# slimgroup/SetIntersectionProjection.jl

Measured on AMD Instinct MI355X. Metric: PARSDMM iterations/sec, higher is better.
Workload: dtype f32

## Files before the change

### setintersectionprojection.jl_amd/csrc/kernels_proj.hip

```cpp
#include <cstdlib>
#include <cstring>
#include <stdexcept>
#include <string>
#include <type_traits>

#include "sipx_device.h"

namespace sipx {

#if defined(__HIP_DEVICE_COMPILE__) && !defined(__gfx950__)
#error "kernels_proj.hip: the relaxed-atomics hand-offs assume gfx950 (see the comment above); port them to release/acquire first"
#endif

constexpr double L1_CAP = 131072.0;
constexpr int L1_REFINES = 1;
constexpr int L1_REFINES_SLAB = 6;
#ifndef SIPX_SPEC_CAP
#define SIPX_SPEC_CAP 1024
#endif
constexpr int SPEC_CAP = SIPX_SPEC_CAP;
constexpr double L1_HW_MAX = 1e-2;
constexpr double L1_CAPDIV = 64.0;
constexpr int L1_WIN_LO = 3, L1_WIN_HI = 4;
__device__ __forceinline__ double l1_probe_mult(int k) {
  const double m[L1_K] = {-64.0, -16.0, -4.0, -1.0, 1.0, 4.0, 16.0, 64.0};
  return m[k];
}
#define SIPX_PASS_GRID launch_blocks(5)
constexpr int SL_ABOVE_S = PREP_SLOTS, SL_ABOVE_C = PREP_SLOTS + 1;
enum { M_FIRST = 0, M_PROBE = 1, M_COMPACT = 2, M_DIST = 3, M_STORE = 4 ,
       M_LEAN = 5  };

template <typename T, int V, int MODE, int SRC>
__global__ __launch_bounds__(BLOCK) void k_pass(Grid G, SetArgs<T> a, int v_is_s, const T* __restrict__ varr,
                                                long long len, ProjScalars<T>* ps, T* __restrict__ compact,
                                                double* __restrict__ partials, T* __restrict__ maxpart) {
  if (MODE == M_PROBE && !(ps->need && !ps->spec_ok && ps->refine)) return;
  long long* cidx = nullptr;
  if (MODE == M_COMPACT && a.prox == PX_CARD) cidx = ps->cidx;
  if (MODE == M_COMPACT && !(ps->need && !ps->spec_ok)) return;
  constexpr bool GATHERS = MODE == M_FIRST || MODE == M_COMPACT || MODE == M_LEAN;
  __shared__ T sbuf[GATHERS ? SPEC_CAP : 1];
  __shared__ unsigned int scnt, sused;
  __shared__ int sovf;
  __shared__ unsigned long long sbase;
  double acc[PREP_SLOTS];
#pragma unroll
  for (int k = 0; k < PREP_SLOTS; ++k) acc[k] = 0;
  ProbeAcc<T> pa;
  if ((a.prox == PX_L1 || a.prox == PX_CARD) && (MODE <= M_PROBE || MODE == M_LEAN)) {
#pragma unroll
    for (int k = 0; k < L1_K; ++k) pa.t[k] = (T)ps->t[k];
  }
  double r_lo = 0, r_hi = -1;
  if ((MODE == M_FIRST || MODE == M_LEAN) && a.prox == PX_L1 && !(a.flags & F_NOSPEC)) { r_lo = ps->spec_lo; r_hi = ps->spec_hi; }
  if (MODE == M_COMPACT) { r_lo = ps->lo; r_hi = ps->hi; }
  const bool gather = r_hi > r_lo;
  const bool lean = (MODE == M_FIRST || MODE == M_LEAN) && a.prox == PX_L1 && gather && ps->lean != 0;
  if (MODE == M_FIRST && lean) return;
  if (MODE == M_LEAN && !lean) return;
  T vmax = T(0), vminp = (T)INFINITY;
  if (GATHERS) {
    if (threadIdx.x == 0) { scnt = 0; sused = 0; sovf = 0; }
    __syncthreads();
  }
  ProxCtx<T> pc;
  if (MODE == M_DIST) pc = make_prox<T>(a.prox, a.plo, a.phi, T(0), ps);
  const int lane = threadIdx.x & 63;

  auto body = [&](T x, long long e, bool live) {
    const T av = fabs(x);
    const double ad = (double)av;
    if (MODE == M_LEAN) {
      pa.add_lean(av, L1_WIN_LO, L1_WIN_HI);
      vminp = (av > T(0) && av < vminp) ? av : vminp;
    } else if (MODE == M_FIRST || MODE == M_PROBE) {
      pa.add(av, x);
      vmax = av > vmax ? av : vmax;
      if (MODE == M_FIRST) vminp = (av > T(0) && av < vminp) ? av : vminp;
    }
    if (MODE == M_COMPACT && ad > r_hi) {
      acc[0] += ad;
      acc[1] += 1.0;
    }
    if (MODE == M_STORE && live) compact[e] = x;
    if (MODE == M_DIST && live) {
      const T pv = prox_apply<T>(pc, x, T(0), T(0), T(0), e);
      const T dlt = pv - x;
      acc[0] += (double)dlt * (double)dlt;
      acc[1] += (double)x * (double)x;
    }
    if (GATHERS && gather) {
      const bool in = ad > r_lo && ad <= r_hi;
      const unsigned long long mask = __ballot(in);
      if (mask) {
        const int leader = __ffsll((long long)mask) - 1;
        const int cnt = __popcll(mask);
        const int my = __popcll(mask & ((1ull << lane) - 1ull));
        unsigned int base = SPEC_CAP;
        if (!cidx) {
          if (lane == leader) base = atomicAdd(&scnt, (unsigned int)cnt);
          base = __shfl(base, leader, 64);
        }
        if (cidx) {
          unsigned long long gb = 0;
          if (lane == leader) gb = atomicAdd(&ps->n_compact, (unsigned long long)cnt);
          gb = __shfl(gb, leader, 64);
          if (in) { compact[gb + my] = av; cidx[gb + my] = e; }
        } else if (base + cnt <= SPEC_CAP) {
          if (in) sbuf[base + my] = av;
          if (lane == leader) atomicMax(&sused, base + (unsigned int)cnt);
        } else if (MODE == M_FIRST || MODE == M_LEAN) {
          sovf = 1;
        } else {
          unsigned long long gb = 0;
          if (lane == leader) gb = atomicAdd(&ps->n_compact, (unsigned long long)cnt);
          gb = __shfl(gb, leader, 64);
          if (in) compact[gb + my] = av;
        }
      }
    }
  };

  auto drain = [&]() {
    if (MODE != M_COMPACT || !gather || cidx) return;
    __syncthreads();
    if (scnt <= SPEC_CAP / 2) return;
    const unsigned int cnt = sused;
    if (threadIdx.x == 0) sbase = cnt ? atomicAdd(&ps->n_compact, (unsigned long long)cnt) : 0ull;
    __syncthreads();
    for (unsigned int i = threadIdx.x; i < cnt; i += BLOCK) compact[sbase + i] = sbuf[i];
    __syncthreads();
    if (threadIdx.x == 0) { scnt = 0; sused = 0; }
    __syncthreads();
  };
  if (SRC == 0) {
    int round = 0;
    for (long long e0 = (long long)blockIdx.x * BLOCK; e0 < len; e0 += (long long)gridDim.x * BLOCK) {
      const long long e = e0 + threadIdx.x;
      body(e < len ? varr[e] : T(0), e, e < len);
      if ((++round & 3) == 0) drain();
    }
  } else {
    const bool ident = a.nblk == 0;
    const int nb = ident ? 1 : a.nblk;
    const bool relax = !(a.gamma == T(1));
    const T gam = a.gamma, omg = T(1) - a.gamma;
    long long v0, nvec;
    vec_range<V>(G, v0, nvec);
    const long long nit = (nvec - v0 + (long long)gridDim.x * BLOCK - 1) / ((long long)gridDim.x * BLOCK);
    for (long long it = 0; it < nit; ++it) {
      const long long vi = v0 + it * (long long)gridDim.x * BLOCK + (long long)blockIdx.x * BLOCK + threadIdx.x;
      const bool live = vi < nvec;
      const long long g = live ? vi * V : v0 * V;
      const Coord c = coords(G, g);
      const Vec<T, V> xc = ldv<T, V>(a.x + g);
      for (int q = 0; q < nb; ++q) {
        const long long e = (long long)q * G.N + g;
        T s[V];
        bool valid[V];
        if (ident) {
#pragma unroll
          for (int k = 0; k < V; ++k) { s[k] = xc.v[k]; valid[k] = true; }
        } else {
          fwd_dir<T, V>(G, a.x, xc, g, c, a.dir[q], a.ih[q], s, valid);
        }
        T out[V];
        if (v_is_s) {
#pragma unroll
          for (int k = 0; k < V; ++k) out[k] = s[k];
        } else {
          const Vec<T, V> yv = ldv<T, V>(a.y + e), lv = ldv<T, V>(a.l + e);
#pragma unroll
          for (int k = 0; k < V; ++k) {
            const T xh = relax ? (gam * s[k] + omg * yv.v[k]) : s[k];
            out[k] = valid[k] ? (xh - lv.v[k] * a.rho1) : T(0);
          }
        }
#pragma unroll
        for (int k = 0; k < V; ++k) body(live ? out[k] : T(0), e + k, live);
      }
      drain();
    }
  }

  if (MODE == M_FIRST || MODE == M_PROBE) {
    pa.to_slots(acc);
    block_reduce_store<PREP_SLOTS>(acc, partials, 0);
    if (MODE == M_FIRST) {
      block_max_store<T>(vmax, maxpart);
      block_min_store<T>(vminp, maxpart + NB);
    }
  } else if (MODE == M_LEAN) {
    double a5[5] = {pa.asum, pa.S[L1_WIN_LO], pa.S[L1_WIN_HI], (double)pa.C[L1_WIN_LO], (double)pa.C[L1_WIN_HI]};
    const int slots[5] = {0, 3 + L1_WIN_LO, 3 + L1_WIN_HI, 3 + L1_K + L1_WIN_LO, 3 + L1_K + L1_WIN_HI};
    block_reduce_store_at<5>(a5, partials, slots);
    block_min_store<T>(vminp, maxpart + NB);
  } else if (MODE == M_COMPACT) {
    double a2[2] = {acc[0], acc[1]};
    block_reduce_store<2>(a2, partials, SL_ABOVE_S);
  } else if (MODE == M_STORE) {
  } else {
    double a2[2] = {acc[0], acc[1]};
    block_reduce_store<2>(a2, partials, 0);
  }
  if (GATHERS && gather) {
    __syncthreads();
    const unsigned int cnt = sused;
    if (threadIdx.x == 0) {
      sbase = cnt ? atomicAdd(&ps->n_compact, (unsigned long long)cnt) : 0ull;
      if ((MODE == M_FIRST || MODE == M_LEAN) && sovf) atomicOr(&ps->spec_overflow, 1);
    }
    __syncthreads();
    for (unsigned int i = threadIdx.x; i < cnt; i += BLOCK) compact[sbase + i] = sbuf[i];
  }
}

template <typename T, int V>
__global__ __launch_bounds__(BLOCK) void k_lean_multi(Grid G, LeanMulti<T> m) {
  __shared__ T sbuf[LEAN_MAX][SPEC_CAP];
  __shared__ unsigned int scnt[LEAN_MAX], sused[LEAN_MAX];
  __shared__ int sovf[LEAN_MAX];
  __shared__ unsigned long long sbase[LEAN_MAX];
  bool on[LEAN_MAX];
  T tlo[LEAN_MAX], thi[LEAN_MAX], vminp[LEAN_MAX];
  double r_lo[LEAN_MAX], r_hi[LEAN_MAX], asum[LEAN_MAX], Slo[LEAN_MAX], Shi[LEAN_MAX];
  unsigned int Clo[LEAN_MAX], Chi[LEAN_MAX];
  bool any = false;
#pragma unroll
  for (int q = 0; q < LEAN_MAX; ++q) {
    on[q] = false;
    tlo[q] = thi[q] = (T)INFINITY; vminp[q] = (T)INFINITY;
    r_lo[q] = 0; r_hi[q] = -1; asum[q] = Slo[q] = Shi[q] = 0; Clo[q] = Chi[q] = 0;
    if (q < m.ns) {
      const ProjScalars<T>* ps = m.s[q].ps;
      r_lo[q] = ps->spec_lo; r_hi[q] = ps->spec_hi;
      on[q] = ps->lean != 0 && r_hi[q] > r_lo[q];
      tlo[q] = (T)ps->t[L1_WIN_LO]; thi[q] = (T)ps->t[L1_WIN_HI];
      any |= on[q];
    }
  }
  if (!any) return;
  if (threadIdx.x < LEAN_MAX) { scnt[threadIdx.x] = 0; sused[threadIdx.x] = 0; sovf[threadIdx.x] = 0; }
  __syncthreads();
  const int lane = threadIdx.x & 63;
  long long v0, nvec;
  vec_range<V>(G, v0, nvec);
  const long long nit = (nvec - v0 + (long long)gridDim.x * BLOCK - 1) / ((long long)gridDim.x * BLOCK);
  const T* x = m.s[0].a.x;
  for (long long it = 0; it < nit; ++it) {
    const long long vi = v0 + it * (long long)gridDim.x * BLOCK + (long long)blockIdx.x * BLOCK + threadIdx.x;
    const bool live = vi < nvec;
    const long long g = live ? vi * V : v0 * V;
    const Coord c = coords(G, g);
    const Vec<T, V> xc = ldv<T, V>(x + g);
#pragma unroll
    for (int q = 0; q < LEAN_MAX; ++q) {
      if (q >= m.ns || !on[q]) continue;
      const SetArgs<T>& a = m.s[q].a;
      const bool ident = a.nblk == 0;
      const int nb = ident ? 1 : a.nblk;
      const bool relax = !(a.gamma == T(1));
      const T gam = a.gamma, omg = T(1) - a.gamma;
      for (int b = 0; b < nb; ++b) {
        const long long e = (long long)b * G.N + g;
        T s[V];
        bool valid[V];
        if (ident) {
#pragma unroll
          for (int k = 0; k < V; ++k) { s[k] = xc.v[k]; valid[k] = true; }
        } else {
          fwd_dir<T, V>(G, a.x, xc, g, c, a.dir[b], a.ih[b], s, valid);
        }
        Vec<T, V> yv = zerov<T, V>(), lv = zerov<T, V>();
        if (!m.v_is_s) { yv = ldv<T, V>(a.y + e); lv = ldv<T, V>(a.l + e); }
#pragma unroll
        for (int k = 0; k < V; ++k) {
          const T xh = relax ? (gam * s[k] + omg * yv.v[k]) : s[k];
          const T vv = m.v_is_s ? (live ? s[k] : T(0)) : (live ? (valid[k] ? (xh - lv.v[k] * a.rho1) : T(0)) : T(0));
          const T av = fabs(vv);
          const double ad = (double)av;
          asum[q] += ad;
          const bool o_lo = av > tlo[q], o_hi = av > thi[q];
          Slo[q] += o_lo ? ad : 0.0; Clo[q] += o_lo ? 1u : 0u;
          Shi[q] += o_hi ? ad : 0.0; Chi[q] += o_hi ? 1u : 0u;
          vminp[q] = (av > T(0) && av < vminp[q]) ? av : vminp[q];
          const bool in = ad > r_lo[q] && ad <= r_hi[q];
          const unsigned long long mask = __ballot(in);
          if (mask) {
            const int leader = __ffsll((long long)mask) - 1;
            const int cnt = __popcll(mask);
            const int my = __popcll(mask & ((1ull << lane) - 1ull));
            unsigned int base = SPEC_CAP;
            if (lane == leader) base = atomicAdd(&scnt[q], (unsigned int)cnt);
            base = __shfl(base, leader, 64);
            if (base + cnt <= SPEC_CAP) {
              if (in) sbuf[q][base + my] = av;
              if (lane == leader) atomicMax(&sused[q], base + (unsigned int)cnt);
            } else {
              sovf[q] = 1;
            }
          }
        }
      }
    }
  }
#pragma unroll
  for (int q = 0; q < LEAN_MAX; ++q) {
    if (q >= m.ns || !on[q]) continue;
    __syncthreads();
    double a5[5] = {asum[q], Slo[q], Shi[q], (double)Clo[q], (double)Chi[q]};
    const int slots[5] = {0, 3 + L1_WIN_LO, 3 + L1_WIN_HI, 3 + L1_K + L1_WIN_LO, 3 + L1_K + L1_WIN_HI};
    block_reduce_store_at<5>(a5, m.s[q].partials, slots);
    block_min_store<T>(vminp[q], m.s[q].maxpart + NB);
    __syncthreads();
    const unsigned int cnt = sused[q];
    if (threadIdx.x == 0) {
      sbase[q] = cnt ? atomicAdd(&m.s[q].ps->n_compact, (unsigned long long)cnt) : 0ull;
      if (sovf[q]) atomicOr(&m.s[q].ps->spec_overflow, 1);
    }
    __syncthreads();
    for (unsigned int i = threadIdx.x; i < cnt; i += BLOCK) m.s[q].compact[sbase[q] + i] = sbuf[q][i];
  }
}

template <typename T>
void K<T>::lean_multi(hipStream_t s, const Grid& g, const LeanMulti<T>& m) {
  if (m.ns < 1 || m.ns > LEAN_MAX || g.n[0] % 4 != 0) throw std::runtime_error("lean_multi: unsupported call");
  double bytes = (double)range_len(g);
  for (int q = 0; q < m.ns; ++q) bytes += (m.v_is_s ? 0.0 : 2.0) * (double)m.s[q].a.nblk_or1() * (double)range_len(g);
  ObsScope obs_(KID_PASS_LEAN, s, bytes * sizeof(T));
  hipLaunchKernelGGL((k_lean_multi<T, 4>), dim3(fit_grid(range_len(g) / 4, SIPX_PASS_GRID)), dim3(BLOCK), 0, s, g, m);
  SIPX_HIP(hipGetLastError());
}


template <typename T, int V, int MODE>
__global__ __launch_bounds__(BLOCK) void k_pass_multi(Grid G, LeanMulti<T> m, int v_is_s) {
  static_assert(MODE == M_FIRST || MODE == M_PROBE || MODE == M_COMPACT, "modes of k_pass_multi");
  constexpr bool GATHERS = MODE == M_FIRST || MODE == M_COMPACT;
  __shared__ T sbuf[GATHERS ? LEAN_MAX : 1][GATHERS ? SPEC_CAP : 1];
  __shared__ unsigned int scnt[LEAN_MAX], sused[LEAN_MAX];
  __shared__ int sovf[LEAN_MAX];
  __shared__ unsigned long long sbase[LEAN_MAX];
  bool on[LEAN_MAX], gather[LEAN_MAX];
  double r_lo[LEAN_MAX], r_hi[LEAN_MAX], above_s[LEAN_MAX], above_c[LEAN_MAX];
  T vmax[LEAN_MAX], vminp[LEAN_MAX];
  ProbeAcc<T> pa[LEAN_MAX];
  bool any = false;
#pragma unroll
  for (int q = 0; q < LEAN_MAX; ++q) {
    on[q] = gather[q] = false;
    r_lo[q] = 0; r_hi[q] = -1; above_s[q] = above_c[q] = 0;
    vmax[q] = T(0); vminp[q] = (T)INFINITY;
    if (q < m.ns) {
      const ProjScalars<T>* ps = m.s[q].ps;
      const SetArgs<T>& a = m.s[q].a;
      const bool l1 = a.prox == PX_L1;
      if (MODE == M_FIRST) {
        if (l1 && !(a.flags & F_NOSPEC)) { r_lo[q] = ps->spec_lo; r_hi[q] = ps->spec_hi; }
        gather[q] = r_hi[q] > r_lo[q];
        on[q] = !(l1 && gather[q] && ps->lean != 0);
      } else if (MODE == M_PROBE) {
        on[q] = l1 && ps->need && !ps->spec_ok && ps->refine;
      } else {
        on[q] = l1 && ps->need && !ps->spec_ok;
        r_lo[q] = ps->lo; r_hi[q] = ps->hi;
        gather[q] = r_hi[q] > r_lo[q];
      }
      if (on[q] && l1 && MODE != M_COMPACT) {
#pragma unroll
        for (int k = 0; k < L1_K; ++k) pa[q].t[k] = (T)ps->t[k];
      }
      any |= on[q];
    }
  }
  if (!any) return;
  if (GATHERS) {
    if (threadIdx.x < LEAN_MAX) { scnt[threadIdx.x] = 0; sused[threadIdx.x] = 0; sovf[threadIdx.x] = 0; }
    __syncthreads();
  }
  const int lane = threadIdx.x & 63;
  long long v0, nvec;
  vec_range<V>(G, v0, nvec);
  const long long nit = (nvec - v0 + (long long)gridDim.x * BLOCK - 1) / ((long long)gridDim.x * BLOCK);
  const T* x = m.s[0].a.x;
  for (long long it = 0; it < nit; ++it) {
    const long long vi = v0 + it * (long long)gridDim.x * BLOCK + (long long)blockIdx.x * BLOCK + threadIdx.x;
    const bool live = vi < nvec;
    const long long g = live ? vi * V : v0 * V;
    const Coord c = coords(G, g);
    const Vec<T, V> xc = ldv<T, V>(x + g);
#pragma unroll
    for (int q = 0; q < LEAN_MAX; ++q) {
      if (q >= m.ns || !on[q]) continue;
      const SetArgs<T>& a = m.s[q].a;
      const bool ident = a.nblk == 0;
      const int nb = ident ? 1 : a.nblk;
      const bool relax = !(a.gamma == T(1));
      const T gam = a.gamma, omg = T(1) - a.gamma;
      for (int b = 0; b < nb; ++b) {
        const long long e = (long long)b * G.N + g;
        T s[V];
        bool valid[V];
        if (ident) {
#pragma unroll
          for (int k = 0; k < V; ++k) { s[k] = xc.v[k]; valid[k] = true; }
        } else {
          fwd_dir<T, V>(G, a.x, xc, g, c, a.dir[b], a.ih[b], s, valid);
        }
        T out[V];
        if (v_is_s) {
#pragma unroll
          for (int k = 0; k < V; ++k) out[k] = s[k];
        } else {
          const Vec<T, V> yv = ldv<T, V>(a.y + e), lv = ldv<T, V>(a.l + e);
#pragma unroll
          for (int k = 0; k < V; ++k) {
            const T xh = relax ? (gam * s[k] + omg * yv.v[k]) : s[k];
            out[k] = valid[k] ? (xh - lv.v[k] * a.rho1) : T(0);
          }
        }
#pragma unroll
        for (int k = 0; k < V; ++k) {
          const T vv = live ? out[k] : T(0);
          const T av = fabs(vv);
          const double ad = (double)av;
          if (MODE == M_FIRST || MODE == M_PROBE) {
            pa[q].add(av, vv);
            vmax[q] = av > vmax[q] ? av : vmax[q];
            if (MODE == M_FIRST) vminp[q] = (av > T(0) && av < vminp[q]) ? av : vminp[q];
          }
          if (MODE == M_COMPACT && ad > r_hi[q]) { above_s[q] += ad; above_c[q] += 1.0; }
          if (GATHERS && gather[q]) {
            const bool in = ad > r_lo[q] && ad <= r_hi[q];
            const unsigned long long mask = __ballot(in);
            if (mask) {
              const int leader = __ffsll((long long)mask) - 1;
              const int cnt = __popcll(mask);
              const int my = __popcll(mask & ((1ull << lane) - 1ull));
              unsigned int base = SPEC_CAP;
              if (lane == leader) base = atomicAdd(&scnt[q], (unsigned int)cnt);
              base = __shfl(base, leader, 64);
              if (base + cnt <= SPEC_CAP) {
                if (in) sbuf[GATHERS ? q : 0][base + my] = av;
                if (lane == leader) atomicMax(&sused[q], base + (unsigned int)cnt);
              } else if (MODE == M_FIRST) {
                sovf[q] = 1;
              } else {
                unsigned long long gb = 0;
                if (lane == leader) gb = atomicAdd(&m.s[q].ps->n_compact, (unsigned long long)cnt);
                gb = __shfl(gb, leader, 64);
                if (in) m.s[q].compact[gb + my] = av;
              }
            }
          }
        }
      }
    }
  }
#pragma unroll
  for (int q = 0; q < LEAN_MAX; ++q) {
    if (q >= m.ns || !on[q]) continue;
    __syncthreads();
    if (MODE == M_FIRST || MODE == M_PROBE) {
      double acc[PREP_SLOTS];
      pa[q].to_slots(acc);
      block_reduce_store<PREP_SLOTS>(acc, m.s[q].partials, 0);
      if (MODE == M_FIRST) {
        __syncthreads();
        block_max_store<T>(vmax[q], m.s[q].maxpart);
        __syncthreads();
        block_min_store<T>(vminp[q], m.s[q].maxpart + NB);
      }
    } else {
      double a2[2] = {above_s[q], above_c[q]};
      block_reduce_store<2>(a2, m.s[q].partials, SL_ABOVE_S);
    }
    if (GATHERS && gather[q]) {
      __syncthreads();
      const unsigned int cnt = sused[q];
      if (threadIdx.x == 0) {
        sbase[q] = cnt ? atomicAdd(&m.s[q].ps->n_compact, (unsigned long long)cnt) : 0ull;
        if (MODE == M_FIRST && sovf[q]) atomicOr(&m.s[q].ps->spec_overflow, 1);
      }
      __syncthreads();
      for (unsigned int i = threadIdx.x; i < cnt; i += BLOCK) m.s[q].compact[sbase[q] + i] = sbuf[GATHERS ? q : 0][i];
    }
  }
}

template <typename T>
void K<T>::pass_multi(int mode, hipStream_t s, const Grid& g, const LeanMulti<T>& m, int v_is_s) {
  if (m.ns < 1 || m.ns > LEAN_MAX || g.n[0] % 4 != 0) throw std::runtime_error("pass_multi: unsupported call");
  double bytes = (double)range_len(g);
  for (int q = 0; q < m.ns; ++q) bytes += (v_is_s ? 0.0 : 2.0) * (double)m.s[q].a.nblk_or1() * (double)range_len(g);
  const dim3 grid(fit_grid(range_len(g) / 4, SIPX_PASS_GRID));
  if (mode == M_FIRST) {
    ObsScope obs_(KID_PASS_FIRST, s, bytes * sizeof(T));
    hipLaunchKernelGGL((k_pass_multi<T, 4, M_FIRST>), grid, dim3(BLOCK), 0, s, g, m, v_is_s);
  } else if (mode == M_PROBE) {
    ObsScope obs_(KID_PASS_PROBE, s, bytes * sizeof(T));
    hipLaunchKernelGGL((k_pass_multi<T, 4, M_PROBE>), grid, dim3(BLOCK), 0, s, g, m, v_is_s);
  } else if (mode == M_COMPACT) {
    ObsScope obs_(KID_PASS_COMPACT, s, bytes * sizeof(T));
    hipLaunchKernelGGL((k_pass_multi<T, 4, M_COMPACT>), grid, dim3(BLOCK), 0, s, g, m, v_is_s);
  } else {
    throw std::runtime_error("pass_multi: unknown mode");
  }
  SIPX_HIP(hipGetLastError());
}

template <typename T>
__global__ void k_ps_init(ProjScalars<T>* ps, long long* cidx) {
  ps->cidx = cidx;
  ps->c_lo = ps->c_hi = 0;
  ps->tau_prev = T(0);
  ps->asum = ps->sumsq = 0;
  ps->vmax = T(0);
  ps->need = 0;
  ps->theta = T(0);
  ps->scale = T(1);
  ps->fill = 0;
  for (int k = 0; k < L1_K; ++k) ps->t[k] = INFINITY;
  ps->lo = ps->hi = 0;
  ps->refine = 0;
  ps->theta_prev = 0;
  ps->n_compact = 0;
  ps->spec_lo = 0;
  ps->spec_hi = -1;
  ps->s_above = ps->c_above = 0;
  ps->hw = 1e-2;
  ps->lean = 0;
  ps->spec_ok = ps->spec_overflow = 0;
  ps->tau = T(0);
  ps->quota = 0x7fffffffffffffffll;
  ps->coop_arrive = ps->coop_finish = ps->coop_abort = 0;
  for (int j = 0; j < SAMPLE_BINS; ++j) ps->hist[j] = 0;
  ps->sampled = ps->dbg_sampled = ps->want_sample = 0;
  ps->samp_ticket = 0;
  ps->pass_ticket = 0;
  ps->gather_overflow = 0;
  ps->rounds_used = 0;
  ps->br_tl = ps->br_Sl = ps->br_Cl = ps->br_th = ps->br_Sh = ps->br_Ch = 0;
  ps->ovf = 0;
  for (int r = 0; r < 2 * SIPX_MAX_WORLD; ++r) ps->mm[r] = 0;
  ps->rescaled = 0;
  ps->resc_bad = 1;
  ps->samp_theta = 0;
  ps->samp_bias = 0;
  ps->samp_bias_ok = 0;
}
template <typename T>
void K<T>::ps_init(hipStream_t s, ProjScalars<T>* ps, long long* cidx) {
  hipLaunchKernelGGL((k_ps_init<T>), dim3(1), dim3(1), 0, s, ps, cidx);
  SIPX_HIP(hipGetLastError());
}

#ifndef SIPX_DECIDE_NT
#define SIPX_DECIDE_NT 256
#endif
template <int NT>
__device__ __forceinline__ void reduce_slots(const double* __restrict__ partials, double* red ) {
  static_assert(NB % NT == 0, "NB must be a multiple of the reducing workgroup");
  constexpr int PER = NB / NT, NW = NT / 64, CH = NT >= 1024 ? PREP_SLOTS : (NT >= 512 ? 8 : 4);
  __shared__ double sm[PREP_SLOTS][NW];
  const int w = threadIdx.x >> 6, lane = threadIdx.x & 63;
#pragma unroll 1
  for (int k0 = 0; k0 < PREP_SLOTS; k0 += CH) {
    double v[CH];
#pragma unroll
    for (int c = 0; c < CH; ++c) {
      double a = 0;
      if (k0 + c < PREP_SLOTS) {
#pragma unroll
        for (int j = 0; j < PER; ++j) a += partials[(long long)(k0 + c) * NB + j * NT + threadIdx.x];
      }
      v[c] = a;
    }
#pragma unroll
    for (int c = 0; c < CH; ++c) {
      const double r = wave_sum(v[c]);
      if (lane == 0 && k0 + c < PREP_SLOTS) sm[k0 + c][w] = r;
    }
  }
  __syncthreads();
  if (threadIdx.x < PREP_SLOTS) {
    double r = 0;
#pragma unroll
    for (int i = 0; i < NW; ++i) r += sm[threadIdx.x][i];
    red[threadIdx.x] = r;
  }
}

template <typename T>
__device__ __forceinline__ T next_up(T v);
template <>
__device__ __forceinline__ float next_up<float>(float v) { return nextafterf(v, INFINITY); }
template <>
__device__ __forceinline__ double next_up<double>(double v) { return nextafter(v, (double)INFINITY); }
template <typename T>
__device__ __forceinline__ void place_probes(ProjScalars<T>* ps, double lo, double hi, double tl, double th) {
  T prev = (T)tl;
  const T top = (T)th;
  for (int k = 0; k < L1_K; ++k) {
    T tc = (T)(lo + (hi - lo) * (double)k / (double)(L1_K - 1));
    if (!(tc > prev)) tc = next_up<T>(prev);
    if (tc < top) { ps->t[k] = (double)tc; prev = tc; }
    else ps->t[k] = INFINITY;
  }
}
template <typename T, int STAGE>
__device__ void decide_body(ProjScalars<T>* ps, int prox, T pmin, T pmax, long long true_len, int nospec, int world,
                            double cap_max, const double* reg);

template <typename T, int STAGE, bool FUSE>
__global__ __launch_bounds__(BLOCK) void k_slot_sums(const double* __restrict__ partials, const T* __restrict__ maxpart,
                                                     ProjScalars<T>* ps, int rank, int world, double* __restrict__ reg, DecideArgs da) {
  if (STAGE == 1 && !(ps->need && !ps->spec_ok && ps->refine)) {
    return;
  }
  __shared__ double sreg[PREP_SLOTS + 1 + 2 * SIPX_MAX_WORLD];
  __shared__ unsigned int sh_ticket;
  auto finish = [&]() {
    __builtin_amdgcn_s_waitcnt(0);
    __syncthreads();
    if (threadIdx.x == 0) sh_ticket = __hip_atomic_fetch_add(&ps->pass_ticket, 1u, __ATOMIC_RELAXED, __HIP_MEMORY_SCOPE_AGENT);
    __syncthreads();
    if (sh_ticket != gridDim.x - 1) return;
    const int nreg = PREP_SLOTS + 1 + 2 * world;
    for (int i = threadIdx.x; i < nreg; i += BLOCK) sreg[i] = __hip_atomic_load(&reg[i], __ATOMIC_RELAXED, __HIP_MEMORY_SCOPE_AGENT);
    __syncthreads();
    if (threadIdx.x != 0) return;
    __hip_atomic_store(&ps->pass_ticket, 0u, __ATOMIC_RELAXED, __HIP_MEMORY_SCOPE_AGENT);
    decide_body<T, STAGE>(ps, da.prox, (T)da.pmin, (T)da.pmax, da.true_len, da.nospec, world, da.cap_max, sreg);
// ... 1555 lines not shown
```

### setintersectionprojection.jl_amd/csrc/sipx_common.h

```cpp
#pragma once
#include <hip/hip_runtime.h>
#include <stdint.h>
#include <cstdio>

#include "env_knobs.h"

namespace sipx {

constexpr int BLOCK = 256;
constexpr int NB = 2048;
constexpr int NB_7 = 1792;
inline int fit_grid(long long nvec, int cap) {
  const long long need = (nvec + BLOCK - 1) / BLOCK;
  return (int)(need < 1 ? 1 : (need < cap ? need : cap));
}
template <typename... P>
inline bool aligned16(const P*... p) {
  return (((reinterpret_cast<uintptr_t>(p) & 15u) == 0) && ...);
}
inline int launch_blocks(int per_cu) {
  static const int cus = [] {
    int dev = 0, n = 0;
    if (hipGetDevice(&dev) != hipSuccess || hipDeviceGetAttribute(&n, hipDeviceAttributeMultiprocessorCount, dev) != hipSuccess || n <= 0)
      n = 256;
    return n;
  }();
  const int g = per_cu * cus;
  return g < 256 ? 256 : (g > NB_7 ? NB_7 : g);
}
constexpr int MAXD = 32;
constexpr int MAX_SETS = 16;
constexpr int QT_N = 4 * 27;
constexpr int YL_SLOTS = 13;
constexpr int L1_K = 8;
#define SIPX_SOLVE_SLOTS 64
#define SIPX_MAX_WORLD 64
constexpr int GATHER_HDR = 8;
constexpr int PREP_SLOTS = 3 + 2 * L1_K;
template <typename T>
constexpr int fast_hdr() { return ((PREP_SLOTS + 4) * 8 / (int)sizeof(T) + 3) / 4 * 4; }
constexpr int SAMPLE_BINS = 1024;
constexpr int SAMPLE_MBITS = 7;

enum KernelId {
  KID_CDS_SPMV = 0, KID_CDS_DOT, KID_CDS_RESID, KID_CDS_FUSED, KID_SQ_SPMV, KID_SQ_DOT, KID_SQ_RESID, KID_CG_BEGIN, KID_CG_XR, KID_CG_P,
  KID_Q_UPDATE, KID_FIN_SUM, KID_RHS, KID_YL, KID_YL_MULTI, KID_ADJ_NORM, KID_LOG3, KID_PASS_FIRST, KID_PASS_LEAN, KID_PASS_PROBE,
  KID_PASS_COMPACT, KID_PASS_DIST, KID_PASS_STORE, KID_PASS_MULTI, KID_SLOT_SUMS, KID_DECIDE, KID_SAMPLE, KID_L1_SOLVE, KID_GATHER,
  KID_PS_RESCALE, KID_CARD, KID_EXT, KID_BB_RULE, KID_OTHER, KID_MF_FWD, KID_MF_ADJ, KID_L21_NORMS, KID_L21_FRAMES, KID_L21_SCALE,
  KID_L21J_NORMS, KID_L21J_FINISH, KID_L21J_SCALE, KID_L21W_PASS, KID_L21W_SCALE,
  KID_L21G_NORMS, KID_L21G_FINISH, KID_L21G_SCALE, KID_TNV_GRAM, KID_TNV_FINISH, KID_TNV_APPLY, KID_L1W_PASS, KID_L1W_APPLY,
  KID_CARDG_RANK, KID_CARDG_ZERO, KID_L20_FRAMES, KID_L20_ZERO, KID_L21S_NORMS, KID_L21S_SCALE,
  KID_L2INF_CLIP, KID_L2INFS_CLIP, KID_L2INF_SCALE, KID_COUNT
};
inline const char* kernel_name(int k) {
  static const char* const names[KID_COUNT] = {
      "k_cds<MODE=0>", "k_cds<MODE=1>", "k_cds<MODE=2>", "k_cds_fused", "k_sq<MODE=0>", "k_sq<MODE=1>", "k_sq<MODE=2>", "k_cg_begin",
      "k_cg_update_xr", "k_cg_update_p", "k_q_update", "k_fin_sum", "k_rhs", "k_yl", "k_yl_multi", "k_adj_norm", "k_log3",
      "k_pass<M_FIRST>", "k_pass<M_LEAN>", "k_pass<M_PROBE>", "k_pass<M_COMPACT>", "k_pass<M_DIST>", "k_pass<M_STORE>", "k_pass_multi",
      "k_slot_sums", "k_decide", "k_sample", "k_l1_solve", "k_gather_pack/unpack", "k_ps_rescale", "k_card_*", "ext_proj (library-backed)",
      "k_bb_rule", "other", "k_mf_fwd", "k_mf_adj", "k_l21_norms", "k_l21_frames", "k_l21_scale",
      "k_l21j_norms", "k_l21j_finish", "k_l21j_scale", "k_l21w_part", "k_l21w_scale",
      "k_l21g_norms", "k_l21g_finish", "k_l21g_scale", "k_tnv_gram", "k_tnv_finish", "k_tnv_apply", "k_l1w_part", "k_l1w_apply",
      "k_cardg_rank", "k_cardg_zero", "k_l20_frames", "k_l20_zero", "k_l21s_norms", "k_l21s_scale",
      "k_l2inf_clip", "k_l2infs_clip", "k_l2inf_scale"};
  return (k >= 0 && k < KID_COUNT) ? names[k] : "?";
}
enum RouteId {
  RT_CDS_MARCH_BANDS = 0,
  RT_CDS_MARCH_TABLE = 4,
  RT_CDS_FLAT = 8,
  RT_CDS_FUSED_FLAT = 11,
  RT_RHS_MARCH = 12,
  RT_RHS_FLAT = 13,
  RT_COUNT = 14
};
inline const char* route_name(int r) {
  static const char* const names[RT_COUNT] = {
      "k_cds_march<MODE=0>/bands", "k_cds_march<MODE=1>/bands", "k_cds_march<MODE=2>/bands", "k_cds_march<MODE=3>/bands",
      "k_cds_march<MODE=0>/table", "k_cds_march<MODE=1>/table", "k_cds_march<MODE=2>/table", "k_cds_march<MODE=3>/table",
      "k_cds<MODE=0>", "k_cds<MODE=1>", "k_cds<MODE=2>", "k_cds_fused", "k_rhs_march", "k_rhs"};
  return (r >= 0 && r < RT_COUNT) ? names[r] : "?";
}
struct LaunchObserver {
  void* user;
  void (*begin)(void* user, int kid, hipStream_t s, double bytes_survey, double bytes_moved);
  void (*end)(void* user, int kid, hipStream_t s);
  void (*route)(void* user, int route);
};
const LaunchObserver*& launch_observer();

struct ObsScope {
  const LaunchObserver* o;
  int kid;
  hipStream_t s;
  ObsScope(int kid_, hipStream_t s_, double bytes_survey, double bytes_moved = -1.0) : o(launch_observer()), kid(kid_), s(s_) {
    if (env_knobs().trace_kernels) fprintf(stderr, "[sipx trace] %s\n", kernel_name(kid));
    if (o) o->begin(o->user, kid, s, bytes_survey, bytes_moved < 0 ? bytes_survey : bytes_moved);
  }
  ~ObsScope() {
    if (o) o->end(o->user, kid, s);
    if (env_knobs().trace_kernels) {
      (void)hipStreamSynchronize(s);
      fprintf(stderr, "[sipx trace]   done\n");
    }
  }
  void route(int r) const { if (o && o->route) o->route(o->user, r); }
  ObsScope(const ObsScope&) = delete;
  ObsScope& operator=(const ObsScope&) = delete;
};

enum { SL_RPRI = 0, SL_DY = 1, SL_HL = 2, SL_HH = 3, SL_LH = 4, SL_DL = 5, SL_GG = 6, SL_GL = 7,
       SL_FE = 8, SL_SS = 9, SL_OBJ = 10, SL_EVO = 11, SL_XX = 12,
       SL_ADJ = 13 , SL_FE2 = 14, SL_SS2 = 15  };
constexpr int SET_SLOTS = 16;

enum { F_FEAS = 1, F_BB = 2, F_FIRST = 4, F_NOSPEC = 8 ,
       F_STORE_DY = 16  };

enum { PX_BOUNDS = 0, PX_BOUNDS_VEC = 1, PX_L1 = 2, PX_L2 = 3, PX_ANNULUS = 4, PX_CARD = 5, PX_PROX_L1 = 6,
       PX_EXT = 8,
       PX_DIST = 100 };

struct Grid {
  long long n[3];
  long long N;
  long long st[3];
  unsigned m1 = 0, s1 = 0, m2 = 0, s2 = 0;
  long long e0 = 0, e1 = -1, s0 = 0;
  void set_fast_div() {
    auto magic = [](long long d, unsigned& m, unsigned& sh) {
      m = 0; sh = 0;
      if (d < 2 || d >= (1ll << 31)) return;
      int l = 0;
      while ((1ll << l) < d) ++l;
      const unsigned long long q = ((unsigned long long)1 << (31 + l)) / (unsigned long long)d + 1ull;
      m = (unsigned)q;
      sh = (unsigned)(l - 1);
    };
    magic(n[0], m1, s1);
    magic(n[1], m2, s2);
  }
};

inline long long range_len(const Grid& g) { return (g.e1 < 0 ? g.N : g.e1) - g.e0; }

struct CdsArgs {
  int d;
  long long off[MAXD];
  int sym = 0;
  int partner[MAXD] = {};
  int march = 0;
  int mb[4] = {0, 0, 0, 0};
  long long gn[3] = {0, 0, 0};
  const void* qtab = nullptr;
};

template <typename T>
struct StencilQ {
  T w0, w[3];
  int mask;
};

template <typename T>
struct ProjScalars {
  double asum;
  double sumsq;
  T vmax;
  T vmin;
  int need;
  T theta;
  T scale;
  int fill;
  double t[L1_K];
  double lo, hi;
  int refine;
  int rounds_used;
  double theta_prev;
  unsigned long long n_compact;
  double spec_lo, spec_hi;
  double s_above, c_above;
  double hw;
  int spec_ok, spec_overflow;
  double dbg[4];
  T tau;
  long long quota;
  long long* cidx;
  double c_lo, c_hi;
  double br_tl, br_Sl, br_Cl, br_th, br_Sh, br_Ch;
  T tau_prev;
  double red[PREP_SLOTS];
  double ovf;
  double mm[2 * SIPX_MAX_WORLD];
  int gather_overflow;
  int lean;
  double coop_hi[2][SIPX_SOLVE_SLOTS], coop_lo[2][SIPX_SOLVE_SLOTS], coop_c[2][SIPX_SOLVE_SLOTS];
  unsigned coop_arrive, coop_finish, coop_abort;
  unsigned long long hist[SAMPLE_BINS];
  unsigned pass_ticket;
  unsigned samp_ticket;
  int rescaled, resc_bad;
  int want_sample;
  int sampled;
  int dbg_sampled;
  double samp_theta;
  double samp_bias;
  int samp_bias_ok;
  double samp_lo, samp_hi, samp_c;
};

struct ChainHooks {
  int world = 1, rank = 0;
  void* user = nullptr;
  void (*allreduce_sum)(void* user, double* buf, size_t count, hipStream_t s) = nullptr;
  void (*allgather)(void* user, void* buf, size_t chunk, int dtype_is_f64, hipStream_t s) = nullptr;
  void* gbuf = nullptr;
  long long gcap = 0;
  long long fcap = 0;
};

struct SampleCtl {
  int enable = 0;
  long long runs = 0;
  int* host_want = nullptr;
  int* host_ovf = nullptr;
  unsigned* verdict = nullptr;
  unsigned seq = 0;
  int lean_done = 0;
  int lean_known = 0;
  long long compact_cap = 0;
};

template <typename T>
struct SetArgs {
  T *y, *l, *dy, *lh0, *y0, *s0, *l0;
  T *yo, *lo;
  T* v;
  const T *x, *m, *xold, *lb, *ub;
  int nblk;
  int dir[3];
  T ih[3];
  T rho, rho1, gamma;
  int prox;
  T plo, phi;
  const ProjScalars<T>* ps;
  int flags;
  int vsrc;
  int nblk_or1() const { return nblk > 0 ? nblk : 1; }
};

struct DecideArgs {
  int prox, nospec;
  double pmin, pmax, cap_max;
  long long true_len;
};
constexpr int SPEC_MAX_SETS = 8;
template <typename T>
struct SpecPackSet {
  const ProjScalars<T>* ps;
  const double* partials;
  const T* maxpart;
  const T* compact;
  T* seg;
  int is_l1;
};
template <typename T>
struct SpecPackArgs {
  int nsets;
  int local = 0;
  long long cap;
  SpecPackSet<T> s[SPEC_MAX_SETS];
};
template <typename T>
struct SpecFinishSet {
  ProjScalars<T>* ps;
  DecideArgs da;
  double* reg;
  const T* fseg0;
  T* compact;
  const double* partials;
  T radius;
  int* host_want;
  unsigned* verdict;
};
template <typename T>
struct SpecFinishArgs {
  int local = 0;
  int nsets, world;
  long long fchunk;
  unsigned seq;
  SpecFinishSet<T> s[SPEC_MAX_SETS];
};

template <typename T>
struct SampleSet {
  SetArgs<T> a;
  ProjScalars<T>* ps;
  double* partials;
  double* reg;
  long long true_len;
};
template <typename T>
struct SampleMulti {
  int v_is_s = 0;
  int ns;
  SampleSet<T> s[SPEC_MAX_SETS];
};
template <typename T>
struct RescaleMulti {
  int n;
  ProjScalars<T>* ps[SPEC_MAX_SETS];
  double factor[SPEC_MAX_SETS];
};

template <typename T>
struct LeanSet {
  SetArgs<T> a;
  ProjScalars<T>* ps;
  T* compact;
  double* partials;
  T* maxpart;
};
constexpr int LEAN_MAX = 3;
template <typename T>
struct LeanMulti {
  int v_is_s = 0;
  int ns;
  LeanSet<T> s[LEAN_MAX];
};

constexpr int MULTI_MAXB = 8;
template <typename T>
struct MultiBlk {
  const T *y, *l;
  T *yo, *lo;
  T *lh0, *s0;
  const T *y0, *l0;
  const ProjScalars<T>* ps;
  int dir;
  int set;
  int first, last;
  int dist;
  int feas_el;
  int in_rhs = 1;
  T ih, rho, rho1, gamma;
  int prox;
  T plo, phi;
};
template <typename T>
struct MultiArgs {
  int nblk;
  MultiBlk<T> b[MULTI_MAXB];
  const T *x, *m, *xold;
  const T* x0;
  T* x0w;
  T* rhs;
  double* partials;
  int flags;
  long long zlo, zhi;
  long long zsum;
};

template <typename T>
struct MkSet {
  T alpha;
  int nblk, comp;
  int dir[3];
  T ih[3];
};
template <typename T>
struct MkArgs {
  int nsets;
  MkSet<T> s[MAX_SETS];
};

template <typename T>
struct QSet {
  T alpha;
  const T* ata;
  int nblk;
  int dir[3];
  T ih[3];
  int nband;
  long long off[9];
// ... 177 lines not shown
```

Baseline: 887.0.

## Specialize lean multi-set pass on compile-time set/direction layouts

```diff
diff --git a/setintersectionprojection.jl_amd/csrc/kernels_proj.hip b/setintersectionprojection.jl_amd/csrc/kernels_proj.hip
--- a/setintersectionprojection.jl_amd/csrc/kernels_proj.hip
+++ b/setintersectionprojection.jl_amd/csrc/kernels_proj.hip
@@ -324,13 +324,251 @@
   }
 }
 
+constexpr unsigned lean_set_code(int nb, int d0, int d1 = 0, int d2 = 0) { return (unsigned)(nb | (d0 << 2) | (d1 << 4) | (d2 << 6)); }
+constexpr unsigned lean_layout(unsigned s0, unsigned s1 = 0, unsigned s2 = 0) {
+  return (unsigned)(1 + (s1 != 0) + (s2 != 0)) | (s0 << 2) | (s1 << 10) | (s2 << 18);
+}
+constexpr int ll_sets(unsigned L) { return (int)(L & 3u); }
+constexpr int ll_nblk(unsigned L, int q) { return (int)((L >> (2 + 8 * q)) & 3u); }
+constexpr int ll_dir(unsigned L, int q, int b) { return (int)((L >> (4 + 8 * q + 2 * b)) & 3u); }
+constexpr int ll_blocks(unsigned L) { return ll_nblk(L, 0) + ll_nblk(L, 1) + ll_nblk(L, 2); }
+constexpr int ll_set_of(unsigned L, int j) { return j < ll_nblk(L, 0) ? 0 : (j < ll_nblk(L, 0) + ll_nblk(L, 1) ? 1 : 2); }
+constexpr int ll_mask_blocks(unsigned L, int mask) {
+  int n = 0;
+  for (int q = 0; q < 3; ++q) n += ((mask >> q) & 1) ? ll_nblk(L, q) : 0;
+  return n;
+}
+constexpr int ll_mask_nth(unsigned L, int mask, int i) {
+  for (int j = 0; j < ll_blocks(L); ++j)
+    if ((mask >> ll_set_of(L, j)) & 1) { if (i == 0) return j; --i; }
+  return 0;
+}
+constexpr int ll_blk_of(unsigned L, int j) { return j - (ll_set_of(L, j) > 0 ? ll_nblk(L, 0) : 0) - (ll_set_of(L, j) > 1 ? ll_nblk(L, 1) : 0); }
+template <typename T, int V>
+constexpr int lean_depth(unsigned L, bool vs) {
+  const int per_block = (vs ? 1 : 3) * V * (int)(sizeof(T) / 4), room = 96 - 40 - 9 * ll_sets(L) - V * (int)(sizeof(T) / 4);
+  const int d = room / per_block;
+  return d < 1 ? 1 : (d > ll_blocks(L) ? ll_blocks(L) : d);
+}
+constexpr unsigned LL_DX_DY_DZ = lean_layout(lean_set_code(1, 0), lean_set_code(1, 1), lean_set_code(1, 2));
+constexpr unsigned LL_TV3 = lean_layout(lean_set_code(3, 2, 1, 0));
+constexpr unsigned LL_TV2 = lean_layout(lean_set_code(2, 1, 0));
+constexpr unsigned LL_DX_DZ3 = lean_layout(lean_set_code(1, 0), lean_set_code(1, 2));
+constexpr unsigned LL_DX_DZ2 = lean_layout(lean_set_code(1, 0), lean_set_code(1, 1));
+#ifndef SIPX_LEAN_LAYOUT
+#define SIPX_LEAN_LAYOUT 1
+#endif
+
+template <int I, int N, typename F>
+__device__ __forceinline__ void static_for(F&& f) {
+  if constexpr (I < N) {
+    f(std::integral_constant<int, I>{});
+    static_for<I + 1, N>(f);
+  }
+}
+
+template <typename T, int V, unsigned L, bool VS>
+__global__ __launch_bounds__(BLOCK, 5) void k_lean_multi_lay(Grid G, LeanMulti<T> m) {
+  constexpr int NS = ll_sets(L), NBT = ll_blocks(L), DEPTH = lean_depth<T, V>(L, VS);
+  __shared__ T sbuf[NS][SPEC_CAP];
+  __shared__ unsigned int scnt[NS], sused[NS];
+  __shared__ int sovf[NS];
+  __shared__ unsigned long long sbase[NS];
+  bool on[NS];
+  T tlo[NS], thi[NS], vminp[NS];
+  double r_lo[NS], r_hi[NS], asum[NS], Slo[NS], Shi[NS];
+  unsigned int Clo[NS], Chi[NS];
+  int mask_on = 0;
+#pragma unroll
+  for (int q = 0; q < NS; ++q) {
+    vminp[q] = (T)INFINITY;
+    asum[q] = Slo[q] = Shi[q] = 0; Clo[q] = Chi[q] = 0;
+    const ProjScalars<T>* ps = m.s[q].ps;
+    r_lo[q] = ps->spec_lo; r_hi[q] = ps->spec_hi;
+    on[q] = ps->lean != 0 && r_hi[q] > r_lo[q];
+    tlo[q] = (T)ps->t[L1_WIN_LO]; thi[q] = (T)ps->t[L1_WIN_HI];
+    mask_on |= on[q] ? (1 << q) : 0;
+  }
+  if (!mask_on) return;
+  if (threadIdx.x < NS) { scnt[threadIdx.x] = 0; sused[threadIdx.x] = 0; sovf[threadIdx.x] = 0; }
+  __syncthreads();
+  const int lane = threadIdx.x & 63;
+  long long v0, nvec;
+  vec_range<V>(G, v0, nvec);
+  const long long nit = (nvec - v0 + (long long)gridDim.x * BLOCK - 1) / ((long long)gridDim.x * BLOCK);
+  const T* x = m.s[0].a.x;
+  const unsigned tv = blockIdx.x * BLOCK + threadIdx.x;
+  const long long stv[3] = {1, G.st[1], G.st[2]};
+  const int ndv[3] = {(int)G.n[0], (int)G.n[1], (int)G.n[2]};
+  T ih[NS][3], rho1[NS], gam[NS], omg[NS];
+  bool relax[NS];
+#pragma unroll
+  for (int q = 0; q < NS; ++q) {
+    const SetArgs<T>& a = m.s[q].a;
+#pragma unroll
+    for (int b = 0; b < 3; ++b) ih[q][b] = a.ih[b];
+    rho1[q] = a.rho1;
+    relax[q] = !(a.gamma == T(1));
+    gam[q] = a.gamma; omg[q] = T(1) - a.gamma;
+  }
+
+  auto trips = [&](auto mc) {
+    constexpr int MASK = decltype(mc)::value, NA = ll_mask_blocks(L, MASK);
+    for (long long it = 0; it < nit; ++it) {
+      const unsigned vi = (unsigned)(v0 + it * (long long)gridDim.x * BLOCK) + tv;
+      const bool live = vi < (unsigned)nvec;
+      const unsigned gu = live ? vi * V : (unsigned)v0 * V;
+      const long long g = gu;
+      Coord c;
+      {
+        const unsigned u = gu, jk = __umulhi(u, G.m1) >> G.s1, kk = __umulhi(jk, G.m2) >> G.s2;
+        c.i = (int)(u - jk * (unsigned)G.n[0]); c.j = (int)(jk - kk * (unsigned)G.n[1]); c.k = (int)kk;
+      }
+      const Vec<T, V> xc = ldv<T, V>(x + g);
+      Vec<T, V> xn[NBT], yv[NBT], lv[NBT];
+      auto issue = [&](auto ic) {
+        constexpr int j = ll_mask_nth(L, MASK, decltype(ic)::value), q = ll_set_of(L, j), b = ll_blk_of(L, j);
+        {
+          if constexpr (ll_dir(L, q, b) == 0) {
+#pragma unroll
+            for (int k = 0; k + 1 < V; ++k) xn[j].v[k] = xc.v[k + 1];
+            xn[j].v[V - 1] = x[g + V];
+          } else {
+            xn[j] = ldv_u<T, V>(x + g + stv[ll_dir(L, q, b)]);
+          }
+          if constexpr (!VS) {
+            const long long e = (long long)b * G.N + g;
+            yv[j] = ldv<T, V>(m.s[q].a.y + e);
+            lv[j] = ldv<T, V>(m.s[q].a.l + e);
+          }
+        }
+      };
+      static_for<0, (DEPTH < NA ? DEPTH : NA)>(issue);
+      static_for<0, NA>([&](auto ic) {
+        constexpr int i = decltype(ic)::value, j = ll_mask_nth(L, MASK, i), q = ll_set_of(L, j), b = ll_blk_of(L, j);
+        {
+          {
+            constexpr int dir = ll_dir(L, q, b);
+            const int cd = coord_of(c, dir);
+            T av[V];
+            bool in[V], anyin = false;
+#pragma unroll
+            for (int k = 0; k < V; ++k) {
+              const bool valid = (cd + (dir == 0 ? k : 0)) < ndv[dir] - 1;
+              const T nih = -ih[q][b];
+              const T d = nih * xc.v[k] + ih[q][b] * xn[j].v[k];
+              const T s = valid ? d : T(0);
+              T vv;
+              if constexpr (VS) {
+                vv = live ? s : T(0);
+              } else {
+                const T xr = gam[q] * s + omg[q] * yv[j].v[k];
+                const T xh = relax[q] ? xr : s;
+                const T w = xh - lv[j].v[k] * rho1[q];
+                vv = (live && valid) ? w : T(0);
+              }
+              av[k] = fabs(vv);
+              const double ad = (double)av[k];
+              asum[q] += ad;
+              const bool o_lo = av[k] > tlo[q], o_hi = av[k] > thi[q];
+              Slo[q] += o_lo ? ad : 0.0; Clo[q] += o_lo ? 1u : 0u;
+              Shi[q] += o_hi ? ad : 0.0; Chi[q] += o_hi ? 1u : 0u;
+              vminp[q] = (av[k] > T(0) && av[k] < vminp[q]) ? av[k] : vminp[q];
+              in[k] = ad > r_lo[q] && ad <= r_hi[q];
+              anyin |= in[k];
+            }
+            if (__ballot(anyin)) {
+#pragma unroll
+              for (int k = 0; k < V; ++k) {
+                const unsigned long long mask = __ballot(in[k]);
+                if (mask) {
+                  const int leader = __ffsll((long long)mask) - 1;
+                  const int cnt = __popcll(mask);
+                  const int my = (int)__builtin_amdgcn_mbcnt_hi((unsigned)(mask >> 32), __builtin_amdgcn_mbcnt_lo((unsigned)mask, 0u));
+                  unsigned int base = SPEC_CAP;
+                  if (lane == leader) base = atomicAdd(&scnt[q], (unsigned int)cnt);
+                  base = __shfl(base, leader, 64);
+                  if (base + cnt <= SPEC_CAP) {
+                    if (in[k]) sbuf[q][base + my] = av[k];
+                    if (lane == leader) atomicMax(&sused[q], base + (unsigned int)cnt);
+                  } else {
+                    sovf[q] = 1;
+                  }
+                }
+              }
+            }
+          }
+        }
+        if constexpr (i + DEPTH < NA) issue(std::integral_constant<int, i + DEPTH>{});
+      });
+    }
+  };
+  static_for<1, (1 << NS)>([&](auto mc) {
+    if (mask_on == decltype(mc)::value) trips(mc);
+  });
+
+  static_for<0, NS>([&](auto qc) {
+    constexpr int q = decltype(qc)::value;
+    if (!on[q]) return;
+    __syncthreads();
+    double a5[5] = {asum[q], Slo[q], Shi[q], (double)Clo[q], (double)Chi[q]};
+    const int slots[5] = {0, 3 + L1_WIN_LO, 3 + L1_WIN_HI, 3 + L1_K + L1_WIN_LO, 3 + L1_K + L1_WIN_HI};
+    block_reduce_store_at<5>(a5, m.s[q].partials, slots);
+    block_min_store<T>(vminp[q], m.s[q].maxpart + NB);
+    __syncthreads();
+    const unsigned int cnt = sused[q];
+    if (threadIdx.x == 0) {
+      sbase[q] = cnt ? atomicAdd(&m.s[q].ps->n_compact, (unsigned long long)cnt) : 0ull;
+      if (sovf[q]) atomicOr(&m.s[q].ps->spec_overflow, 1);
+    }
+    __syncthreads();
+    for (unsigned int i = threadIdx.x; i < cnt; i += BLOCK) m.s[q].compact[sbase[q] + i] = sbuf[q][i];
+  });
+}
+
+template <typename T>
+static unsigned lean_layout_of(const LeanMulti<T>& m) {
+  unsigned code = (unsigned)m.ns;
+  for (int q = 0; q < m.ns; ++q) {
+    const SetArgs<T>& a = m.s[q].a;
+    if (a.nblk < 1 || a.nblk > 3) return 0u;
+    unsigned sc = (unsigned)a.nblk;
+    for (int b = 0; b < a.nblk; ++b) {
+      if (a.dir[b] < 0 || a.dir[b] > 2) return 0u;
+      sc |= (unsigned)a.dir[b] << (2 + 2 * b);
+    }
+    code |= sc << (2 + 8 * q);
+    if (m.s[q].a.x != m.s[0].a.x) return 0u;
+  }
+  return code;
+}
+template <typename T, unsigned L>
+static void lean_layout_launch(hipStream_t s, const Grid& g, const LeanMulti<T>& m, int blocks) {
+  if (m.v_is_s)
+    hipLaunchKernelGGL((k_lean_multi_lay<T, 4, L, true>), dim3(blocks), dim3(BLOCK), 0, s, g, m);
+  else
+    hipLaunchKernelGGL((k_lean_multi_lay<T, 4, L, false>), dim3(blocks), dim3(BLOCK), 0, s, g, m);
+}
+
 template <typename T>
 void K<T>::lean_multi(hipStream_t s, const Grid& g, const LeanMulti<T>& m) {
   if (m.ns < 1 || m.ns > LEAN_MAX || g.n[0] % 4 != 0) throw std::runtime_error("lean_multi: unsupported call");
   double bytes = (double)range_len(g);
   for (int q = 0; q < m.ns; ++q) bytes += (m.v_is_s ? 0.0 : 2.0) * (double)m.s[q].a.nblk_or1() * (double)range_len(g);
   ObsScope obs_(KID_PASS_LEAN, s, bytes * sizeof(T));
-  hipLaunchKernelGGL((k_lean_multi<T, 4>), dim3(fit_grid(range_len(g) / 4, SIPX_PASS_GRID)), dim3(BLOCK), 0, s, g, m);
+  const int blocks = fit_grid(range_len(g) / 4, SIPX_PASS_GRID);
+  bool lay = true;
+  switch ((SIPX_LEAN_LAYOUT && g.m1 != 0 && g.m2 != 0) ? lean_layout_of(m) : 0u) {
+    case LL_DX_DY_DZ: lean_layout_launch<T, LL_DX_DY_DZ>(s, g, m, blocks); break;
+    case LL_TV3: lean_layout_launch<T, LL_TV3>(s, g, m, blocks); break;
+    case LL_TV2: lean_layout_launch<T, LL_TV2>(s, g, m, blocks); break;
+    case LL_DX_DZ3: lean_layout_launch<T, LL_DX_DZ3>(s, g, m, blocks); break;
+    case LL_DX_DZ2: lean_layout_launch<T, LL_DX_DZ2>(s, g, m, blocks); break;
+    default:
+      lay = false;
+      hipLaunchKernelGGL((k_lean_multi<T, 4>), dim3(blocks), dim3(BLOCK), 0, s, g, m);
+  }
+  obs_.route(lay ? RT_LEAN_LAYOUT : RT_LEAN_GENERIC);
   SIPX_HIP(hipGetLastError());
 }
 
diff --git a/setintersectionprojection.jl_amd/csrc/sipx_common.h b/setintersectionprojection.jl_amd/csrc/sipx_common.h
--- a/setintersectionprojection.jl_amd/csrc/sipx_common.h
+++ b/setintersectionprojection.jl_amd/csrc/sipx_common.h
@@ -72,13 +72,16 @@
   RT_CDS_FUSED_FLAT = 11,
   RT_RHS_MARCH = 12,
   RT_RHS_FLAT = 13,
-  RT_COUNT = 14
+  RT_LEAN_LAYOUT = 14,
+  RT_LEAN_GENERIC = 15,
+  RT_COUNT = 16
 };
 inline const char* route_name(int r) {
   static const char* const names[RT_COUNT] = {
       "k_cds_march<MODE=0>/bands", "k_cds_march<MODE=1>/bands", "k_cds_march<MODE=2>/bands", "k_cds_march<MODE=3>/bands",
       "k_cds_march<MODE=0>/table", "k_cds_march<MODE=1>/table", "k_cds_march<MODE=2>/table", "k_cds_march<MODE=3>/table",
-      "k_cds<MODE=0>", "k_cds<MODE=1>", "k_cds<MODE=2>", "k_cds_fused", "k_rhs_march", "k_rhs"};
+      "k_cds<MODE=0>", "k_cds<MODE=1>", "k_cds<MODE=2>", "k_cds_fused", "k_rhs_march", "k_rhs",
+      "k_lean_multi/layout", "k_lean_multi/generic"};
   return (r >= 0 && r < RT_COUNT) ? names[r] : "?";
 }
 struct LaunchObserver {
```

Measured after the change: 894.5, median of 6. About the same (+0.9%).
